# qdrant/quantization

Measured on AMD Instinct MI355X. Metric: scored vectors/sec, 10Mx768 u8 dot, higher is better.
Workload: dtype u8; 1 GPU; 10000000 x 768 store: f32 U[0,1) -> scalar u8 (dot); per step: encode_query + score_all over the shard; quantizer=u8, rows_per_gpu=10000000, dim=768, distance=dot, exchange=scores, gather_group=1, launch=single rank, world_size_seen=1, encode_ahead=False, total_rows=10000000, queries=16

## Files before the change

include/quantization_amd.h:

```cpp
#ifndef QUANTIZATION_AMD_H
#define QUANTIZATION_AMD_H

#include <stddef.h>
#include <stdint.h>

#ifdef __cplusplus
extern "C" {
#endif

#define QAMD_API __attribute__((visibility("default")))

typedef enum {
    QAMD_OK = 0,
    QAMD_ERR_IO = 1,
    QAMD_ERR_ENCODING = 2,
    QAMD_ERR_ARGUMENTS = 3,
    QAMD_ERR_STOPPED = 4,
    QAMD_ERR_OUT_OF_RANGE = 5,
    QAMD_ERR_DEVICE = 6
} qamd_status;

typedef enum { QAMD_DOT = 0, QAMD_L1 = 1, QAMD_L2 = 2 } qamd_distance;

typedef enum { QAMD_MEM_HOST = 0, QAMD_MEM_DEVICE = 1 } qamd_mem;

typedef struct {
    uint64_t dim;
    uint64_t count;
    int32_t distance_type;
    int32_t invert;
} qamd_vector_parameters;

typedef int (*qamd_stop_fn)(void *user);

QAMD_API const char *qamd_last_error(void);
QAMD_API const char *qamd_version(void);
QAMD_API int qamd_device_count(void);
QAMD_API qamd_status qamd_set_device(int device);
QAMD_API int qamd_get_device(void);
QAMD_API void qamd_thread_release(void);

typedef struct qamd_u8 qamd_u8;
typedef struct qamd_u8_query qamd_u8_query;

typedef struct {
    uint64_t actual_dim;
    float alpha;
    float offset;
    float multiplier;
    qamd_vector_parameters vector_parameters;
} qamd_u8_metadata;

QAMD_API uint64_t qamd_u8_quantized_vector_size(const qamd_vector_parameters *vp);
QAMD_API uint64_t qamd_u8_actual_dim(const qamd_vector_parameters *vp);

QAMD_API qamd_status qamd_u8_encode(const float *data, qamd_mem data_mem,
                                    const qamd_vector_parameters *vp, const float *quantile,
                                    const float *alpha_offset, qamd_stop_fn stop, void *stop_user,
                                    void *stream, qamd_u8 **out);

typedef struct qamd_u8_encoder qamd_u8_encoder;
QAMD_API qamd_status qamd_u8_encoder_begin(const qamd_vector_parameters *vp, const float *quantile,
                                           const float *alpha_offset, qamd_stop_fn stop, void *stop_user,
                                           void *stream, qamd_u8_encoder **out);
QAMD_API qamd_status qamd_u8_encoder_observe(qamd_u8_encoder *e, const float *batch, uint64_t n_rows,
                                             qamd_mem batch_mem);
QAMD_API qamd_status qamd_u8_encoder_push(qamd_u8_encoder *e, const float *batch, uint64_t n_rows,
                                          qamd_mem batch_mem);
QAMD_API qamd_status qamd_u8_encoder_finish(qamd_u8_encoder *e, qamd_u8 **out);
QAMD_API void qamd_u8_encoder_abort(qamd_u8_encoder *e);

QAMD_API qamd_status qamd_u8_find_min_max(const float *data, qamd_mem data_mem, uint64_t n_rows, uint64_t dim,
                                          void *stream, float *min, float *max);
QAMD_API qamd_status qamd_u8_find_quantile_interval(const float *data, qamd_mem data_mem, uint64_t count, uint64_t dim,
                                                    float quantile, void *stream, int *found, float *min, float *max);

QAMD_API qamd_status qamd_u8_from_rows(const uint8_t *rows, qamd_mem rows_mem,
                                       const qamd_u8_metadata *meta, void *stream, qamd_u8 **out);

QAMD_API qamd_status qamd_u8_export_rows(const qamd_u8 *h, uint8_t *rows, qamd_mem rows_mem,
                                         void *stream);
QAMD_API qamd_status qamd_u8_export_rows_range(const qamd_u8 *h, uint64_t first_row, uint64_t n_rows,
                                               uint8_t *rows, qamd_mem rows_mem, void *stream);
QAMD_API qamd_status qamd_u8_get_metadata(const qamd_u8 *h, qamd_u8_metadata *out);

QAMD_API qamd_status qamd_u8_save(const qamd_u8 *h, const char *data_path, const char *meta_path);
QAMD_API qamd_status qamd_u8_load(const char *data_path, const char *meta_path,
// ... 329 lines not shown
```

quantization_amd/csrc/common.hpp:

```cpp
#pragma once

#include <hip/hip_runtime.h>

#include <atomic>
#include <mutex>
#include <cstdarg>
#include <cstdint>
#include <cstdlib>
#include <cstdio>
#include <cstring>
#include <string>
#include <vector>

#include "json.hpp"

#include "../../include/quantization_amd.h"

namespace qamd {

std::string &last_error();
qamd_status fail(qamd_status st, const char *fmt, ...) __attribute__((format(printf, 2, 3)));

#define QAMD_HIP(expr)                                                                      \
    do {                                                                                    \
// ... 20 lines not shown
    DeviceGuard &operator=(const DeviceGuard &) = delete;
    qamd_status status() const { return st_; }

  private:
    int prev_ = -1;
    bool switched_ = false;
    qamd_status st_ = QAMD_OK;
};
#define QAMD_ON_DEVICE(dev)                  \
    ::qamd::DeviceGuard _qamd_dev_guard(dev); \
    QAMD_TRY(_qamd_dev_guard.status())

inline const char *dev_env(const char *name) {
#ifdef QAMD_DEV
    return getenv(name);
#else
    (void)name;
    return nullptr;
#endif
}
inline uint64_t dev_env_u64(const char *name, uint64_t dflt) {
    const char *e = dev_env(name);
    if (!e || !*e) return dflt;
    char *end = nullptr;
    const unsigned long long v = strtoull(e, &end, 10);
    return (*end == 0 && v > 0) ? (uint64_t)v : dflt;
}
inline uint64_t stage_bytes(uint64_t dflt) {
    static const uint64_t v = dev_env_u64("QAMD_DEV_STAGE_BYTES", 0);
    return v ? v : dflt;
}
inline bool host_whole_allowed() {
    static const bool on = [] { const char *e = dev_env("QAMD_DEV_HOST_WHOLE"); return !(e && e[0] == '0'); }();
    return on;
}
inline uint64_t pq_planar_max_rows() {
    static const uint64_t v = dev_env_u64("QAMD_DEV_PQ_PLANAR_ROWS", 1ull << 28);
    return v;
}
inline uint64_t pq_skew_max_rows() {
    static const uint64_t v = dev_env_u64("QAMD_DEV_PQ_SKEW_ROWS", 1ull << 30);
    return v;
}

class DeviceOnce {
  public:
    template <class F> qamd_status run(F &&setup) {
        int dev = 0;
        if (hipGetDevice(&dev) != hipSuccess || dev < 0 || dev > 63) return setup();
        const uint64_t bit = 1ull << dev;
        if (done_.load(std::memory_order_acquire) & bit) return QAMD_OK;
        std::lock_guard<std::mutex> g(mu_);
        if (done_.load(std::memory_order_relaxed) & bit) return QAMD_OK;
        const qamd_status st = setup();
        if (st == QAMD_OK) done_.fetch_or(bit, std::memory_order_release);
        return st;
    }

  private:
    std::atomic<uint64_t> done_{0};
    std::mutex mu_;
};
#define QAMD_LDS_OPT_IN(kernel, bytes)                                                                            \
    do {                                                                                                          \
        static ::qamd::DeviceOnce _qamd_once;                                                                     \
        QAMD_TRY(_qamd_once.run([]() -> qamd_status {                                                             \
// ... 105 lines not shown
```

quantization_amd/csrc/u8.hip:

```cpp
#include <algorithm>
#include <cmath>
#include <cstdlib>
#include <memory>
#include <vector>

#include "common.hpp"
#include "lists.hpp"
#include "multi_reduce.hpp"
#include "topk.hpp"
#include "topk_device.hpp"
#include "u8_internal.hpp"

#pragma clang fp contract(off)

using namespace qamd;

namespace {

constexpr int kBlock = 256;
constexpr int kScanBlock = 512;
constexpr uint64_t kRowPad = 1024;
constexpr uint64_t kQuantileSample = 100000;

enum Epilogue : int { EPI_POINT = 0, EPI_INTERNAL = 1 };
// ... 59 lines not shown
}
template <int G> __device__ __forceinline__ float avx2_lane_sum(uint32_t (&acc)[8]) {
    float f[8];
#pragma unroll
    for (int k = 0; k < 8; k++) f[k] = (float)(int32_t)group_sum<G>(acc[k]);
    float a0 = f[0] + f[4], a1 = f[1] + f[5], a2 = f[2] + f[6], a3 = f[3] + f[7];
    return (a0 + a2) + (a1 + a3);
}

__device__ __forceinline__ uint32_t f32_to_u8(float v, float alpha, float offset) {
    float x = (v - offset) / alpha;
    x = (x < 0.0f) ? 0.0f : x;
    x = (x > 127.0f) ? 127.0f : x;
    return (x != x) ? 0u : (uint32_t)x;
}

__device__ __forceinline__ bool quant_decided(float y) {
    constexpr float kBand = 3.0517578125e-05f;
    const float fr = __builtin_amdgcn_fractf(y);
    return (__builtin_fabsf(fr - 0.5f) <= 0.5f - kBand) || (__builtin_fabsf(y - 64.0f) >= 64.0f + kBand);
}
__device__ __forceinline__ uint32_t quant_code(float y) {
    return (uint32_t)__builtin_amdgcn_fmed3f(y, 0.0f, 127.0f);
}
__device__ __forceinline__ uint32_t f32x4_to_u8x4_fast(const float4 &f, float alpha, float offset, float r_alpha) {
    const float y0 = (f.x - offset) * r_alpha, y1 = (f.y - offset) * r_alpha, y2 = (f.z - offset) * r_alpha,
                y3 = (f.w - offset) * r_alpha;
    if (quant_decided(y0) && quant_decided(y1) && quant_decided(y2) && quant_decided(y3))
        return quant_code(y0) | (quant_code(y1) << 8) | (quant_code(y2) << 16) | (quant_code(y3) << 24);
    return f32_to_u8(f.x, alpha, offset) | (f32_to_u8(f.y, alpha, offset) << 8) | (f32_to_u8(f.z, alpha, offset) << 16) |
           (f32_to_u8(f.w, alpha, offset) << 24);
}

template <int G, int ITERS, int UNROLL, bool IS_L1, bool EXACT, bool FILTER>
__global__ __launch_bounds__(kScanBlock) void u8_scan_kernel(
    const uint4 *__restrict__ codes, const float *__restrict__ offsets,
    const uint4 *__restrict__ qcodes, const float *__restrict__ q_off_p, float multiplier,
    uint32_t n_rows, uint32_t row_chunks, float *__restrict__ out, TopkFilter filt) {
    constexpr int RW = 64 / G;
    constexpr int TILE = RW * UNROLL;
    const int lane = threadIdx.x & 63;
    const int sub = lane % G;
    const int rslot = lane / G;
    const uint64_t wave = ((uint64_t)blockIdx.x * kScanBlock + threadIdx.x) >> 6;
    const uint64_t base = wave * TILE;
    if (base >= n_rows) return;

    uint4 v[UNROLL][ITERS];
#pragma unroll
    for (int u = 0; u < UNROLL; u++) {
        const uint64_t row = base + u * RW + rslot;
        const uint4 *p = codes + row * row_chunks;
#pragma unroll
        for (int it = 0; it < ITERS; it++) {
            const uint32_t c = sub + it * G;
            if (EXACT) {
                v[u][it] = ld_nt(p + c);
            } else {
                const uint32_t cc = c < row_chunks ? c : row_chunks - 1;
                uint4 t = ld_nt(p + cc);
                const bool in = c < row_chunks;
                v[u][it] = make_uint4(in ? t.x : 0, in ? t.y : 0, in ? t.z : 0, in ? t.w : 0);
            }
        }
    }
    uint4 q[ITERS];
#pragma unroll
    for (int it = 0; it < ITERS; it++) {
        const uint32_t c = sub + it * G;
        if (EXACT) {
            q[it] = qcodes[c];
        } else {
            const uint4 t = qcodes[c < row_chunks ? c : row_chunks - 1];
            const bool in = c < row_chunks;
            q[it] = make_uint4(in ? t.x : 0, in ? t.y : 0, in ? t.z : 0, in ? t.w : 0);
        }
    }
    const float q_off = *q_off_p;
    constexpr int NGROUPS = (UNROLL + G - 1) / G;
    float v_off[NGROUPS];
#pragma unroll
    for (int g = 0; g < NGROUPS; g++)
        v_off[g] = offsets[base + (uint64_t)(g * G + sub) * RW + rslot];
    float mine = 0.0f;
    uint32_t pivot = 0;
    if (FILTER) pivot = *filt.pivot_key;
#pragma unroll
    for (int u = 0; u < UNROLL; u++) {
        uint32_t acc = 0;
#pragma unroll
        for (int it = 0; it < ITERS; it++)
            acc = IS_L1 ? sad16(v[u][it], q[it], acc) : dot16(v[u][it], q[it], acc);
        acc = group_sum<G>(acc);
        if (sub == (u % G)) mine = epilogue(multiplier, acc, q_off, v_off[u / G], 0.0f, EPI_POINT);
        if ((u % G) == G - 1 || u == UNROLL - 1) {
            constexpr int dummy = 0;
            (void)dummy;
            const int first = (u / G) * G;
            const uint64_t row = base + (uint64_t)(first + sub) * RW + rslot;
            if (sub <= u - first && row < n_rows) {
                if (FILTER) topk_offer(filt, pivot, mine, (uint32_t)row);
                else __builtin_nontemporal_store(mine, out + row);
            }
        }
    }
}

template <int G, int ITERS, int UNROLL, int NQ, bool IS_L1, bool EXACT, bool FILTER>
__global__ __launch_bounds__(kScanBlock) void u8_scan_multi_kernel(
    const uint4 *__restrict__ codes, const float *__restrict__ offsets, const uint8_t *__restrict__ qcodes,
    uint32_t q_pitch, const float *__restrict__ q_offs, uint32_t nq_valid ,
    float multiplier, uint32_t n_rows, uint32_t row_chunks, float *__restrict__ out ,
    uint64_t out_pitch, TopkFilterSlices slices) {
    static_assert(G >= NQ, "one lane of the row group per query");
    constexpr int RW = 64 / G;
    constexpr int TILE = RW * UNROLL;
    constexpr int TPW = NQ;
    const int lane = threadIdx.x & 63;
    const int sub = lane % G, rslot = lane / G;
    const uint64_t wave = ((uint64_t)blockIdx.x * kScanBlock + threadIdx.x) >> 6;
    if (wave * TILE * TPW >= n_rows) return;
    uint4 q[NQ][ITERS];
#pragma unroll
    for (int j = 0; j < NQ; j++) {
        const uint4 *qj = reinterpret_cast<const uint4 *>(qcodes + (size_t)((uint32_t)j < nq_valid ? j : nq_valid - 1) * q_pitch);
// ... 649 lines not shown
    }
}

__global__ __launch_bounds__(kBlock) void split_rows_kernel(const uint32_t *__restrict__ rows32,
                                                           uint64_t n_rows, uint32_t row_dwords,
                                                           uint32_t *__restrict__ codes32,
                                                           float *__restrict__ offsets) {
    const uint64_t total = n_rows * row_dwords;
    const uint64_t stride = (uint64_t)gridDim.x * kBlock;
    for (uint64_t t = (uint64_t)blockIdx.x * kBlock + threadIdx.x; t < total; t += stride) {
        uint64_t r = t / row_dwords;
        uint32_t k = (uint32_t)(t - r * row_dwords);
        uint32_t w = rows32[t];
        if (k == 0)
            offsets[r] = __uint_as_float(w);
        else
            codes32[r * (row_dwords - 1) + (k - 1)] = w;
    }
}

__global__ __launch_bounds__(kBlock) void join_rows_kernel(const uint32_t *__restrict__ codes32,
                                                          const float *__restrict__ offsets,
                                                          uint64_t n_rows, uint32_t row_dwords,
                                                          uint32_t *__restrict__ rows32) {
    const uint64_t total = n_rows * row_dwords;
    const uint64_t stride = (uint64_t)gridDim.x * kBlock;
    for (uint64_t t = (uint64_t)blockIdx.x * kBlock + threadIdx.x; t < total; t += stride) {
        uint64_t r = t / row_dwords;
        uint32_t k = (uint32_t)(t - r * row_dwords);
        rows32[t] = k == 0 ? __float_as_uint(offsets[r]) : codes32[r * (row_dwords - 1) + (k - 1)];
    }
}

int grid_for(uint64_t work_items, uint64_t per_block, int blocks_per_cu) {
    uint64_t want = (work_items + per_block - 1) / per_block;
    uint64_t cap = (uint64_t)device_info().cu_count * blocks_per_cu;
    if (want < 1) want = 1;
    return (int)(want > cap ? cap : want);
}

float host_multiplier(float alpha, int distance, int invert) {
    float m = distance == QAMD_DOT ? alpha * alpha : distance == QAMD_L1 ? alpha : -2.0f * alpha * alpha;
    return invert ? -m : m;
}

uint64_t actual_dim_of(uint64_t dim) { return dim + (16 - dim % 16) % 16; }

}


namespace {

qamd_status alloc_store(qamd_u8 *h) {
    h->padded_rows = round_up(h->count, kRowPad) + kRowPad;
    h->row_chunks = (uint32_t)(h->meta.actual_dim / 16);
    QAMD_TRY(h->codes.alloc_zero_tail(h->padded_rows * h->meta.actual_dim, h->count * h->meta.actual_dim));
    QAMD_TRY(h->offsets.alloc_zero_tail(h->padded_rows * sizeof(float), h->count * sizeof(float)));
    return QAMD_OK;
}

template <bool IS_L1> struct ScanLaunch {
    template <int G, int ITERS, int UNROLL>
    static void go(const qamd_u8 *h, const uint4 *qc, const float *qo, float *out, const TopkFilter *filt,
                   hipStream_t s) {
        constexpr int TILE = (64 / G) * UNROLL;
        const uint64_t waves = (h->count + TILE - 1) / TILE;
        const unsigned grid = (unsigned)((waves + kScanBlock / 64 - 1) / (kScanBlock / 64));
        const bool exact = h->row_chunks == (uint32_t)(G * ITERS);
#define QAMD_U8_GO(EX, FI)                                                                                  \
    hipLaunchKernelGGL((u8_scan_kernel<G, ITERS, UNROLL, IS_L1, EX, FI>), dim3(grid), dim3(kScanBlock), 0, s, \
                       h->codes.as<uint4>(), h->offsets.as<float>(), qc, qo, h->meta.multiplier,            \
                       (uint32_t)h->count, h->row_chunks, out, filt ? *filt : TopkFilter{})
        if (filt) {
            if (exact) QAMD_U8_GO(true, true);
            else QAMD_U8_GO(false, true);
        } else {
            if (exact) QAMD_U8_GO(true, false);
            else QAMD_U8_GO(false, false);
        }
#undef QAMD_U8_GO
    }
};

template <bool IS_L1>
bool launch_scan(const qamd_u8 *h, const uint4 *qc, const float *qo, float *out, const TopkFilter *filt,
                 hipStream_t s) {
    using L = ScanLaunch<IS_L1>;
    const uint32_t rc = h->row_chunks;
    if (rc == 1) return L::template go<1, 1, 4>(h, qc, qo, out, filt, s), true;
    if (rc == 2) return L::template go<2, 1, 4>(h, qc, qo, out, filt, s), true;
    if (rc <= 4) return L::template go<4, 1, 8>(h, qc, qo, out, filt, s), true;
    if (rc <= 8) return L::template go<8, 1, 8>(h, qc, qo, out, filt, s), true;
    switch ((rc + 15) / 16) {
        case 1: return L::template go<16, 1, 8>(h, qc, qo, out, filt, s), true;
        case 2: return L::template go<16, 2, 4>(h, qc, qo, out, filt, s), true;
        case 3: return L::template go<16, 3, 4>(h, qc, qo, out, filt, s), true;
        case 4: return L::template go<16, 4, 2>(h, qc, qo, out, filt, s), true;
        case 5: return L::template go<16, 5, 2>(h, qc, qo, out, filt, s), true;
        case 6: return L::template go<16, 6, 2>(h, qc, qo, out, filt, s), true;
        case 7: return L::template go<16, 7, 2>(h, qc, qo, out, filt, s), true;
        case 8: return L::template go<16, 8, 2>(h, qc, qo, out, filt, s), true;
        default: break;
    }
    return false;
}

template <bool IS_L1>
void launch_scan_generic(const qamd_u8 *h, const uint4 *qc, const float *qo, float *out, hipStream_t s) {
    uint64_t waves = (h->count + 3) / 4;
    unsigned grid = (unsigned)((waves + kBlock / 64 - 1) / (kBlock / 64));
    hipLaunchKernelGGL((u8_scan_generic_kernel<IS_L1>), dim3(grid), dim3(kBlock), 0, s,
                       h->codes.as<uint4>(), h->offsets.as<float>(), qc, qo, h->meta.multiplier,
                       (uint32_t)h->count, h->row_chunks, out);
}

template <bool IS_L1> struct SmallLaunch {
    template <int G, int ITERS>
    static qamd_status go(const qamd_u8 *h, const uint4 *qc, const float *qo, const FusedQuery *fq, const SmallTopkPlan &pl,
                          const SmallTopk &p, hipStream_t s) {
        const bool exact = h->row_chunks == (uint32_t)(G * ITERS);
        if constexpr (G * ITERS * 16 > (int)kFusedQueryDims + 15 * 16) {
            if (fq) return fail(QAMD_ERR_ARGUMENTS, "fused query does not fit the kernel arguments");
        } else if (fq) {
            QueryByValue qv;
            memcpy(qv.v, fq->values, (size_t)fq->qdim * 4);
            const qamd_vector_parameters &vp = h->meta.vector_parameters;
#define QAMD_U8_SMALL_FUSED(EX)                                                                                        \
    hipLaunchKernelGGL((u8_topk_small_fused_kernel<G, ITERS, IS_L1, EX>), dim3(pl.workgroups), dim3(1024), 0, s,          \
                       h->codes.as<uint4>(), h->offsets.as<float>(), qv, fq->qdim, (uint32_t)h->meta.actual_dim,         \
                       h->meta.alpha, h->meta.offset, vp.distance_type, vp.invert, fq->qbuf, h->meta.multiplier,           \
                       (uint32_t)h->count, h->row_chunks, pl.rows_per_wg, p)
            if (exact) QAMD_U8_SMALL_FUSED(true);
            else QAMD_U8_SMALL_FUSED(false);
#undef QAMD_U8_SMALL_FUSED
            QAMD_HIP(hipGetLastError());
            return QAMD_OK;
        }
#define QAMD_U8_SMALL(EX)                                                                                       \
    hipLaunchKernelGGL((u8_topk_small_kernel<G, ITERS, IS_L1, EX>), dim3(pl.workgroups), dim3(1024), 0, s,       \
                       h->codes.as<uint4>(), h->offsets.as<float>(), qc, qo, h->meta.multiplier, (uint32_t)h->count, \
                       h->row_chunks, pl.rows_per_wg, p)
        if (exact) QAMD_U8_SMALL(true);
        else QAMD_U8_SMALL(false);
#undef QAMD_U8_SMALL
        QAMD_HIP(hipGetLastError());
        return QAMD_OK;
    }
};

int small_group(uint32_t rc) { return rc == 1 ? 1 : rc == 2 ? 2 : rc <= 4 ? 4 : rc <= 8 ? 8 : rc <= 128 ? 16 : 0; }

template <bool IS_L1>
qamd_status launch_small(const qamd_u8 *h, const uint4 *qc, const float *qo, const FusedQuery *fq, const SmallTopkPlan &pl,
                         const SmallTopk &p, hipStream_t s) {
    using L = SmallLaunch<IS_L1>;
    const uint32_t rc = h->row_chunks;
    if (rc == 1) return L::template go<1, 1>(h, qc, qo, fq, pl, p, s);
    if (rc == 2) return L::template go<2, 1>(h, qc, qo, fq, pl, p, s);
    if (rc <= 4) return L::template go<4, 1>(h, qc, qo, fq, pl, p, s);
    if (rc <= 8) return L::template go<8, 1>(h, qc, qo, fq, pl, p, s);
    switch ((rc + 15) / 16) {
        case 1: return L::template go<16, 1>(h, qc, qo, fq, pl, p, s);
        case 2: return L::template go<16, 2>(h, qc, qo, fq, pl, p, s);
        case 3: return L::template go<16, 3>(h, qc, qo, fq, pl, p, s);
        case 4: return L::template go<16, 4>(h, qc, qo, fq, pl, p, s);
        case 5: return L::template go<16, 5>(h, qc, qo, fq, pl, p, s);
        case 6: return L::template go<16, 6>(h, qc, qo, fq, pl, p, s);
        case 7: return L::template go<16, 7>(h, qc, qo, fq, pl, p, s);
        case 8: return L::template go<16, 8>(h, qc, qo, fq, pl, p, s);
        default: break;
    }
    return fail(QAMD_ERR_ARGUMENTS, "no small top-k kernel for %u chunks", rc);
}

template <bool IS_L1, int G, int ITERS, int UNROLL, int NQ>
void launch_multi_shape(const qamd_u8 *h, const uint8_t *qcodes, uint64_t q_pitch, const float *q_offs, uint32_t nq_valid,
                        float *out, const TopkFilterSlices *slices, hipStream_t s) {
    constexpr int TILE = (64 / G) * UNROLL * NQ;
    const uint64_t waves = (h->count + TILE - 1) / TILE;
    const unsigned grid = (unsigned)((waves + kScanBlock / 64 - 1) / (kScanBlock / 64));
    const bool exact = h->row_chunks == (uint32_t)(G * ITERS);
#define QAMD_U8_MULTI(EX, FI)                                                                                      \
    hipLaunchKernelGGL((u8_scan_multi_kernel<G, ITERS, UNROLL, NQ, IS_L1, EX, FI>), dim3(grid), dim3(kScanBlock), 0, s, \
                       h->codes.as<uint4>(), h->offsets.as<float>(), qcodes, (uint32_t)q_pitch, q_offs, nq_valid,   \
                       h->meta.multiplier, (uint32_t)h->count, h->row_chunks, out, (uint64_t)h->count,             \
                       slices ? *slices : TopkFilterSlices{})
    if (slices) {
        if (exact) QAMD_U8_MULTI(true, true);
        else QAMD_U8_MULTI(false, true);
    } else {
        if (exact) QAMD_U8_MULTI(true, false);
        else QAMD_U8_MULTI(false, false);
    }
#undef QAMD_U8_MULTI
}

bool lane_order(const qamd_u8 *h) {
    return h->lane_mode == 1 && h->meta.vector_parameters.distance_type != QAMD_L1;
}

uint32_t multi_width(const qamd_u8 *h) {
    const uint32_t rc = h->row_chunks, iters = (rc + 15) / 16;
    const bool l1 = h->meta.vector_parameters.distance_type == QAMD_L1;
    if (rc < 9 || iters > 8 || lane_order(h)) return 0;
    return l1 && iters <= 3 ? 8 : iters <= 6 ? 4 : 2;
}

template <bool IS_L1>
bool launch_multi(const qamd_u8 *h, uint32_t nq_valid, const uint8_t *qcodes, uint64_t q_pitch, const float *q_offs,
                  float *out, const TopkFilterSlices *slices, hipStream_t s) {
    const uint32_t iters = (h->row_chunks + 15) / 16, width = multi_width(h);
    if (nq_valid < 2 || nq_valid > width) return false;
#define QAMD_U8_MULTI_IT(IT, UN)                                                                              \
    case IT:                                                                                                  \
        if constexpr (IS_L1 && IT <= 3) {                                                                     \
            if (nq_valid > 4) {                                                                               \
                launch_multi_shape<IS_L1, 16, IT, UN, 8>(h, qcodes, q_pitch, q_offs, nq_valid, out, slices, s); \
                return true;                                                                                  \
            }                                                                                                 \
        }                                                                                                     \
        if (nq_valid > 2) launch_multi_shape<IS_L1, 16, IT, UN, (IT <= 6 ? 4 : 2)>(h, qcodes, q_pitch, q_offs, nq_valid, out, slices, s); \
        else launch_multi_shape<IS_L1, 16, IT, UN, 2>(h, qcodes, q_pitch, q_offs, nq_valid, out, slices, s);  \
        return true;
    switch (iters) {
        QAMD_U8_MULTI_IT(1, 4) QAMD_U8_MULTI_IT(2, 2) QAMD_U8_MULTI_IT(3, 2) QAMD_U8_MULTI_IT(4, 2)
        QAMD_U8_MULTI_IT(5, 1) QAMD_U8_MULTI_IT(6, 1) QAMD_U8_MULTI_IT(7, 1) QAMD_U8_MULTI_IT(8, 1)
        default: break;
    }
#undef QAMD_U8_MULTI_IT
    return false;
}

bool fused_capable(const qamd_u8 *h) { return !lane_order(h) && h->row_chunks <= 128; }

bool u8_small_plan(const qamd_u8 *h, uint32_t k, SmallTopkPlan &plan) {
    const int g = small_group(h->row_chunks);
    if (!g || !fused_capable(h)) return false;
    const uint32_t tile = 2 * (64 / g);
    const uint32_t least = (uint32_t)std::max<uint64_t>(16 * tile, (128 * 1024) / std::max<uint64_t>(h->meta.actual_dim, 1));
    return small_topk_plan(h->count, k, tile, least, plan);
}

qamd_status scan_ptrs(const qamd_u8 *h, const uint4 *qc, const float *qo, float *out_dev, hipStream_t s,
                      const TopkFilter *filt = nullptr) {
    if (h->count == 0) return QAMD_OK;
    const bool is_l1 = h->meta.vector_parameters.distance_type == QAMD_L1;
    if (lane_order(h)) {
        uint64_t waves = (h->count + 3) / 4;
        unsigned grid = (unsigned)((waves + kBlock / 64 - 1) / (kBlock / 64));
        hipLaunchKernelGGL((u8_scan_avx2_lanes_kernel<true>), dim3(grid), dim3(kBlock), 0, s,
                           h->codes.as<uint4>(), h->offsets.as<float>(), qc, qo, h->meta.multiplier,
                           (uint32_t)h->count, h->row_chunks, out_dev);
    } else if (is_l1) {
        if (!launch_scan<true>(h, qc, qo, out_dev, filt, s)) launch_scan_generic<true>(h, qc, qo, out_dev, s);
    } else {
        if (!launch_scan<false>(h, qc, qo, out_dev, filt, s)) launch_scan_generic<false>(h, qc, qo, out_dev, s);
    }
    QAMD_HIP(hipGetLastError());
    return QAMD_OK;
}

qamd_status scan_into(const qamd_u8 *h, const qamd_u8_query *q, float *out_dev, hipStream_t s,
                      const TopkFilter *filt = nullptr) {
    return scan_ptrs(h, reinterpret_cast<const uint4 *>(q->buf.as<uint8_t>() + 16), q->buf.as<float>(), out_dev, s, filt);
}

qamd_status check_query(const qamd_u8 *h, const qamd_u8_query *q) {
    if (!h || !q) return fail(QAMD_ERR_ARGUMENTS, "null handle or query");
    if (q->actual_dim != h->meta.actual_dim)
        return fail(QAMD_ERR_ARGUMENTS, "query has %llu codes, store rows have %llu",
                    (unsigned long long)q->actual_dim, (unsigned long long)h->meta.actual_dim);
    return QAMD_OK;
}

template <bool IS_L1>
qamd_status launch_pairs(const qamd_u8 *h, const uint4 *qc, const float *qo, const uint8_t *q_batch, uint32_t q_pitch,
                         const float *q_offs, const uint32_t *lists, uint32_t n_lists, const uint32_t *list_rows, float diff,
                         int mode, const uint32_t *ids_dev, uint64_t n_ids, float *out_dev, hipStream_t s) {
    const uint64_t ppb = pairs_per_block(n_ids, 16);
// ... 332 lines not shown
            const uint64_t nr = std::min(batch_rows, count - r0);
            const float *src = nullptr;
            QAMD_TRY(batch_src(r0, nr, src));
            QAMD_TRY(acc.feed(src, nr * dim, s));
            if (data_mem == QAMD_MEM_HOST) QAMD_HIP(hipStreamSynchronize(s));
        }
        float mn, mx;
        QAMD_TRY(acc.result(s, mn, mx));
        alpha = (mx - mn) / 127.0f;
        offset = mn;
        if (quantile && !(count < 127 || *quantile >= 1.0f)) {
            bool found = false;
            float qmn = 0.0f, qmx = 0.0f;
            QAMD_TRY(quantile_interval_device(data, data_mem, count, dim, *quantile, s, found, qmn, qmx));
            if (found) {
                alpha = (qmx - qmn) / 127.0f;
                offset = qmn;
            }
        }
    }

    for (uint64_t r0 = 0; r0 < count; r0 += batch_rows) {
        if (stop && stop(stop_user)) return fail(QAMD_ERR_STOPPED, "Stopped");
        const uint64_t nr = std::min(batch_rows, count - r0);
        const float *src = nullptr;
        QAMD_TRY(batch_src(r0, nr, src));
        QAMD_TRY(launch_quantize(h.get(), src, nr, r0, alpha, offset, s));
        if (data_mem == QAMD_MEM_HOST || stop) QAMD_HIP(hipStreamSynchronize(s));
    }
    QAMD_HIP(hipStreamSynchronize(s));
    h->meta.alpha = alpha;
    h->meta.offset = offset;
    h->meta.multiplier = host_multiplier(alpha, vp->distance_type, vp->invert);
    *out = h.release();
    return QAMD_OK;
}

qamd_status qamd_u8_from_rows(const uint8_t *rows, qamd_mem rows_mem, const qamd_u8_metadata *meta,
                              void *stream, qamd_u8 **out) {
    if (!meta || !out) return fail(QAMD_ERR_ARGUMENTS, "null argument");
    const qamd_vector_parameters &vp = meta->vector_parameters;
    if (meta->actual_dim != actual_dim_of(vp.dim))
        return fail(QAMD_ERR_ARGUMENTS, "metadata actual_dim %llu does not match dim %llu",
                    (unsigned long long)meta->actual_dim, (unsigned long long)vp.dim);
    if (vp.count > 0xFFFFFFFFull) return fail(QAMD_ERR_ARGUMENTS, "count exceeds u32 row ids");
    if (vp.count > 0 && !rows) return fail(QAMD_ERR_ARGUMENTS, "rows is null");
    QAMD_ON_DEVICE(current_device());
    hipStream_t s = as_stream(stream);
    std::unique_ptr<qamd_u8> h(new qamd_u8);
    h->device = current_device();
    h->count = vp.count;
    h->meta = *meta;
    QAMD_TRY(alloc_store(h.get()));
    const uint64_t stride = meta->actual_dim + 4;
    const uint32_t row_dwords = (uint32_t)(stride / 4);
    const uint64_t batch_rows = std::max<uint64_t>(1, stage_bytes(256ull << 20) / stride);
    DevBuf stage;
    if (rows_mem == QAMD_MEM_HOST && vp.count)
        QAMD_TRY(stage.alloc(std::min<uint64_t>(batch_rows, vp.count) * stride));
    for (uint64_t r0 = 0; r0 < vp.count; r0 += batch_rows) {
        const uint64_t nr = std::min(batch_rows, vp.count - r0);
        const uint8_t *src = rows + r0 * stride;
        if (rows_mem == QAMD_MEM_HOST) {
            QAMD_TRY(copy_in(stage.ptr, src, QAMD_MEM_HOST, nr * stride, s));
            src = stage.as<uint8_t>();
        }
        int grid = grid_for(nr * row_dwords, kBlock * 4, 8);
        hipLaunchKernelGGL(split_rows_kernel, dim3(grid), dim3(kBlock), 0, s,
                           reinterpret_cast<const uint32_t *>(src), nr, row_dwords,
                           h->codes.as<uint32_t>() + r0 * (row_dwords - 1), h->offsets.as<float>() + r0);
        QAMD_HIP(hipGetLastError());
        if (rows_mem == QAMD_MEM_HOST) QAMD_HIP(hipStreamSynchronize(s));
    }
    QAMD_HIP(hipStreamSynchronize(s));
    *out = h.release();
    return QAMD_OK;
}

qamd_status qamd_u8_export_rows_range(const qamd_u8 *h, uint64_t first_row, uint64_t n_rows, uint8_t *rows,
                                      qamd_mem rows_mem, void *stream) {
    if (!h) return fail(QAMD_ERR_ARGUMENTS, "null handle");
    if (first_row > h->count || n_rows > h->count - first_row)
        return fail(QAMD_ERR_OUT_OF_RANGE, "rows [%llu, +%llu) out of range (count %llu)", (unsigned long long)first_row,
                    (unsigned long long)n_rows, (unsigned long long)h->count);
    if (n_rows == 0) return QAMD_OK;
    if (!rows) return fail(QAMD_ERR_ARGUMENTS, "rows is null");
    QAMD_ON_DEVICE(h->device);
    hipStream_t s = as_stream(stream);
    const uint64_t stride = h->meta.actual_dim + 4;
    const uint32_t row_dwords = (uint32_t)(stride / 4);
    const uint64_t batch_rows = std::max<uint64_t>(1, stage_bytes(256ull << 20) / stride);
    DevBuf stage;
    if (rows_mem == QAMD_MEM_HOST) QAMD_TRY(stage.alloc(std::min<uint64_t>(batch_rows, n_rows) * stride));
    for (uint64_t r0 = 0; r0 < n_rows; r0 += batch_rows) {
        const uint64_t nr = std::min(batch_rows, n_rows - r0), src_row = first_row + r0;
        uint8_t *dst = rows_mem == QAMD_MEM_HOST ? stage.as<uint8_t>() : rows + r0 * stride;
        int grid = grid_for(nr * row_dwords, kBlock * 4, 8);
        hipLaunchKernelGGL(join_rows_kernel, dim3(grid), dim3(kBlock), 0, s,
                           h->codes.as<uint32_t>() + src_row * (row_dwords - 1), h->offsets.as<float>() + src_row, nr,
                           row_dwords, reinterpret_cast<uint32_t *>(dst));
        QAMD_HIP(hipGetLastError());
        if (rows_mem == QAMD_MEM_HOST)
            QAMD_TRY(copy_out(rows + r0 * stride, QAMD_MEM_HOST, dst, nr * stride, s));
    }
    return QAMD_OK;
}

// ... 423 lines not shown
                    (unsigned long long)(e->pushed + n_rows), (unsigned long long)e->vp.count);
    QAMD_ON_DEVICE(e->device);
    QAMD_TRY(encoder_close_pass1(e));
    const uint64_t dim = e->vp.dim;
    const uint64_t piece_rows = std::max<uint64_t>(1, stage_bytes(kStagePieceBytes) / (dim * 4 + 1));
    for (uint64_t r = 0; r < n_rows; r += piece_rows) {
        const uint64_t nr = std::min(piece_rows, n_rows - r);
        const void *src = nullptr;
        bool staged = false;
        QAMD_TRY(local_view(batch + r * dim, batch_mem, nr * dim * 4, e->stage, e->stream, &src, &staged));
        QAMD_TRY(launch_quantize(e->h.get(), static_cast<const float *>(src), nr, e->pushed + r, e->alpha, e->offset,
                                 e->stream));
        if (staged) QAMD_HIP(hipStreamSynchronize(e->stream));
    }
    e->pushed += n_rows;
    return QAMD_OK;
}

qamd_status qamd_u8_encoder_finish(qamd_u8_encoder *e, qamd_u8 **out) {
    if (!e || !out) return fail(QAMD_ERR_ARGUMENTS, "null argument");
    std::unique_ptr<qamd_u8_encoder> own(e);
    if (e->pushed != e->vp.count)
        return fail(QAMD_ERR_ARGUMENTS, "Vector count %llu does not match vector parameters count %llu",
                    (unsigned long long)e->pushed, (unsigned long long)e->vp.count);
    QAMD_ON_DEVICE(e->device);
    QAMD_HIP(hipStreamSynchronize(e->stream));
    if (e->vp.count == 0) {
        e->h->meta.alpha = e->h->meta.offset = e->h->meta.multiplier = 0.0f;
    } else {
        e->h->meta.alpha = e->alpha;
        e->h->meta.offset = e->offset;
        e->h->meta.multiplier = host_multiplier(e->alpha, e->vp.distance_type, e->vp.invert);
    }
    *out = e->h.release();
    return QAMD_OK;
}

void qamd_u8_encoder_abort(qamd_u8_encoder *e) {
    if (!e) return;
    DeviceGuard g(e->device);
    (void)hipStreamSynchronize(e->stream);
    delete e;
}

}

namespace qamd {

qamd_status u8_minmax_range(const float *data, qamd_mem mem, uint64_t n_rows, uint64_t dim, hipStream_t s, float *mn,
                            float *mx) {
    MinMaxAcc acc;
    QAMD_TRY(acc.init(s));
    DevBuf stage;
    const uint64_t piece_rows = std::max<uint64_t>(1, stage_bytes(kStagePieceBytes) / std::max<uint64_t>(dim * 4, 1));
    for (uint64_t r = 0; r < n_rows && dim; r += piece_rows) {
        const uint64_t nr = std::min(piece_rows, n_rows - r);
        const void *src = nullptr;
        bool staged = false;
        QAMD_TRY(local_view(data + r * dim, mem, nr * dim * 4, stage, s, &src, &staged));
        QAMD_TRY(acc.feed(static_cast<const float *>(src), nr * dim, s));
        if (staged) QAMD_HIP(hipStreamSynchronize(s));
    }
    return acc.result(s, *mn, *mx);
}

qamd_status u8_quantile_interval(const float *data, qamd_mem mem, uint64_t count, uint64_t dim, float quantile,
// ... 126 lines not shown
                                          : launch_multi<false>(h, nq, qcodes, pitch, offsets_dev + q, o, nullptr, stream));
        if (ok) {
            q += nq;
        } else {
            QAMD_TRY(scan_ptrs(h, reinterpret_cast<const uint4 *>(qcodes), offsets_dev + q, o, stream));
            q += 1;
        }
    }
    QAMD_HIP(hipGetLastError());
    return QAMD_OK;
}

qamd_status u8_topk_single(const qamd_u8 *h, const uint8_t *codes_dev, const float *offset_dev, uint32_t k,
                           int largest, uint32_t *out_ids, float *out_scores, qamd_mem out_mem, hipStream_t stream) {
    return u8_topk_ptrs(h, codes_dev, offset_dev, k, largest, out_ids, out_scores, out_mem, stream, nullptr);
}

qamd_status u8_score_single(const qamd_u8 *h, const uint8_t *codes_dev, const float *offset_dev, float *out_dev,
                            hipStream_t stream) {
    return scan_ptrs(h, reinterpret_cast<const uint4 *>(codes_dev), offset_dev, out_dev, stream);
}

}

#ifdef QAMD_DEV
extern "C" __attribute__((visibility("default"))) void qamd_dev_u8_ptrs(const qamd_u8 *h, const void **codes,
                                                                        const void **offsets) {
    *codes = h->codes.ptr;
    *offsets = h->offsets.ptr;
}
extern "C" __attribute__((visibility("default"))) const void *qamd_dev_u8_query_ptr(const qamd_u8_query *q) {
    return q->buf.ptr;
}
#endif
```

quantization_amd/csrc/u8_internal.hpp:

```cpp
#pragma once
#include <atomic>
#include <mutex>

#include "common.hpp"
#include "lists.hpp"

struct qamd_u8 {
    int device = 0;
    qamd_u8_metadata meta{};
    uint64_t count = 0;
    uint64_t padded_rows = 0;
    uint32_t row_chunks = 0;
    int lane_mode = 0;
    qamd::DevBuf codes;
    qamd::DevBuf offsets;
    mutable std::mutex sample_mu;
    mutable qamd::DevBuf sample_codes, sample_offsets;
    mutable uint32_t sample_rows = 0;
};

struct qamd_u8_query {
    int device = 0;
    uint64_t actual_dim = 0;
    qamd::DevBuf buf;
    mutable qamd::ReadyEvent ready;
    mutable std::vector<float> host_f32;
    float alpha = 0.0f, offset = 0.0f;
    int distance = 0, invert = 0;
    mutable std::atomic<bool> deferred{false};
    mutable std::mutex encode_mu;
    bool pooled = false;
    mutable std::atomic<bool> async_used{false};
    ~qamd_u8_query() {
        if (pooled) qamd::query_buf_put(buf, !async_used.load(std::memory_order_relaxed) && ready.complete());
    }
};

namespace qamd {
qamd_status u8_minmax_range(const float *data, qamd_mem mem, uint64_t n_rows, uint64_t dim, hipStream_t s, float *mn,
                            float *mx);
qamd_status u8_quantile_interval(const float *data, qamd_mem mem, uint64_t count, uint64_t dim, float quantile,
                                 hipStream_t s, bool *found, float *mn, float *mx);
}

namespace qamd {
qamd_status u8_encode_queries_device(const qamd_u8 *h, const float *queries_dev, uint64_t n_queries, uint64_t qdim,
                                     uint8_t *codes_dev , uint64_t code_pitch,
                                     float *offsets_dev ,
// ... 25 lines not shown
```

Before: 9.085 billion vectors/s.

## Add 7-bit packed code image to shrink u8 scan bandwidth

At encode time, when every stored code fits in 7 bits, builds a second device image that moves the bits of the trailing chunks into the free high bit of the leading chunks. Rows then occupy 7/8 of the original chunk count. The single-query scan kernel gains a PACKED path for Dot and L2. It splits each word into its 7-bit part and its high bits and uses a shifted dot against extra query chunks, cutting bytes read per row in a memory-bound scan. The cost is extra device memory, a synchronous build step, and more ALU work per chunk; the multi-query and small-top-k kernels still read the unpacked codes.

```diff
diff --git a/include/quantization_amd.h b/include/quantization_amd.h
--- a/include/quantization_amd.h
+++ b/include/quantization_amd.h
@@ -53,6 +53,7 @@
 
 QAMD_API uint64_t qamd_u8_quantized_vector_size(const qamd_vector_parameters *vp);
 QAMD_API uint64_t qamd_u8_actual_dim(const qamd_vector_parameters *vp);
+
 
 QAMD_API qamd_status qamd_u8_encode(const float *data, qamd_mem data_mem,
                                     const qamd_vector_parameters *vp, const float *quantile,
diff --git a/quantization_amd/csrc/common.hpp b/quantization_amd/csrc/common.hpp
--- a/quantization_amd/csrc/common.hpp
+++ b/quantization_amd/csrc/common.hpp
@@ -76,6 +76,10 @@
 }
 inline bool host_whole_allowed() {
     static const bool on = [] { const char *e = dev_env("QAMD_DEV_HOST_WHOLE"); return !(e && e[0] == '0'); }();
+    return on;
+}
+inline bool u8_packed_allowed() {
+    static const bool on = [] { const char *e = dev_env("QAMD_DEV_U8_PACKED"); return !(e && e[0] == '0'); }();
     return on;
 }
 inline uint64_t pq_planar_max_rows() {
diff --git a/quantization_amd/csrc/u8.hip b/quantization_amd/csrc/u8.hip
--- a/quantization_amd/csrc/u8.hip
+++ b/quantization_amd/csrc/u8.hip
@@ -115,11 +115,12 @@
            (f32_to_u8(f.w, alpha, offset) << 24);
 }
 
-template <int G, int ITERS, int UNROLL, bool IS_L1, bool EXACT, bool FILTER>
+template <int G, int ITERS, int UNROLL, bool IS_L1, bool EXACT, bool FILTER, bool PACKED = false>
 __global__ __launch_bounds__(kScanBlock) void u8_scan_kernel(
     const uint4 *__restrict__ codes, const float *__restrict__ offsets,
     const uint4 *__restrict__ qcodes, const float *__restrict__ q_off_p, float multiplier,
-    uint32_t n_rows, uint32_t row_chunks, float *__restrict__ out, TopkFilter filt) {
+    uint32_t n_rows, uint32_t row_chunks, uint32_t n_extra, float *__restrict__ out, TopkFilter filt) {
+    static_assert(!(PACKED && IS_L1), "the packed image serves Dot and L2 only");
     constexpr int RW = 64 / G;
     constexpr int TILE = RW * UNROLL;
     const int lane = threadIdx.x & 63;
@@ -139,6 +140,8 @@
             const uint32_t c = sub + it * G;
             if (EXACT) {
                 v[u][it] = ld_nt(p + c);
+            } else if (PACKED) {
+                v[u][it] = ld_nt(p + (it < ITERS - 1 || c < row_chunks ? c : row_chunks - 1));
             } else {
                 const uint32_t cc = c < row_chunks ? c : row_chunks - 1;
                 uint4 t = ld_nt(p + cc);
@@ -159,6 +162,18 @@
             q[it] = make_uint4(in ? t.x : 0, in ? t.y : 0, in ? t.z : 0, in ? t.w : 0);
         }
     }
+    uint4 qx[PACKED ? ITERS : 1];
+    uint32_t qsh[PACKED ? ITERS : 1];
+    if (PACKED) {
+#pragma unroll
+        for (int it = 0; it < ITERS; it++) {
+            const uint32_t c = sub + it * G, e = c / 7;
+            const bool has = c < 7 * n_extra;
+            const uint4 t = qcodes[has ? row_chunks + e : 0];
+            qx[it] = make_uint4(has ? t.x : 0, has ? t.y : 0, has ? t.z : 0, has ? t.w : 0);
+            qsh[it] = 7 - (c - 7 * e);
+        }
+    }
     const float q_off = *q_off_p;
     constexpr int NGROUPS = (UNROLL + G - 1) / G;
     float v_off[NGROUPS];
@@ -172,8 +187,17 @@
     for (int u = 0; u < UNROLL; u++) {
         uint32_t acc = 0;
 #pragma unroll
-        for (int it = 0; it < ITERS; it++)
-            acc = IS_L1 ? sad16(v[u][it], q[it], acc) : dot16(v[u][it], q[it], acc);
+        for (int it = 0; it < ITERS; it++) {
+            if (PACKED) {
+                const uint4 &w = v[u][it];
+                const uint32_t hi = dot16(make_uint4(w.x & 0x80808080u, w.y & 0x80808080u, w.z & 0x80808080u,
+                                                     w.w & 0x80808080u), qx[it], 0);
+                acc = dot16(make_uint4(w.x & 0x7F7F7F7Fu, w.y & 0x7F7F7F7Fu, w.z & 0x7F7F7F7Fu, w.w & 0x7F7F7F7Fu),
+                            q[it], acc) + (hi >> qsh[it]);
+            } else {
+                acc = IS_L1 ? sad16(v[u][it], q[it], acc) : dot16(v[u][it], q[it], acc);
+            }
+        }
         acc = group_sum<G>(acc);
         if (sub == (u % G)) mine = epilogue(multiplier, acc, q_off, v_off[u / G], 0.0f, EPI_POINT);
         if ((u % G) == G - 1 || u == UNROLL - 1) {
@@ -889,6 +913,32 @@
     }
 }
 
+__global__ __launch_bounds__(kBlock) void u8_pack7_kernel(const uint4 *__restrict__ codes, uint64_t n_rows,
+                                                          uint32_t row_chunks, uint32_t pchunks, uint32_t n_extra,
+                                                          uint4 *__restrict__ packed, uint32_t *__restrict__ bad) {
+    const uint64_t total = n_rows * pchunks, stride = (uint64_t)gridDim.x * kBlock;
+    uint32_t high = 0;
+    for (uint64_t t = (uint64_t)blockIdx.x * kBlock + threadIdx.x; t < total; t += stride) {
+        const uint64_t r = t / pchunks;
+        const uint32_t j = (uint32_t)(t - r * pchunks);
+        const uint4 *row = codes + r * row_chunks;
+        const uint4 a = row[j];
+        uint32_t w[4] = {a.x & 0x7F7F7F7Fu, a.y & 0x7F7F7F7Fu, a.z & 0x7F7F7F7Fu, a.w & 0x7F7F7F7Fu};
+        high |= a.x | a.y | a.z | a.w;
+        if (j < 7 * n_extra) {
+            const uint4 x = row[pchunks + j / 7];
+            const uint32_t b = j % 7;
+            high |= x.x | x.y | x.z | x.w;
+            w[0] |= ((x.x >> b) & 0x01010101u) << 7;
+            w[1] |= ((x.y >> b) & 0x01010101u) << 7;
+            w[2] |= ((x.z >> b) & 0x01010101u) << 7;
+            w[3] |= ((x.w >> b) & 0x01010101u) << 7;
+        }
+        packed[t] = make_uint4(w[0], w[1], w[2], w[3]);
+    }
+    if (high & 0x80808080u) atomicOr(bad, 1u);
+}
+
 int grid_for(uint64_t work_items, uint64_t per_block, int blocks_per_cu) {
     uint64_t want = (work_items + per_block - 1) / per_block;
     uint64_t cap = (uint64_t)device_info().cu_count * blocks_per_cu;
@@ -916,24 +966,70 @@
     return QAMD_OK;
 }
 
+qamd_status build_packed(qamd_u8 *h, hipStream_t s) {
+    h->packed.release();
+    h->packed_chunks = 0;
+    const uint32_t rc = h->row_chunks, n_extra = rc / 8, pchunks = rc - n_extra;
+    if (!u8_packed_allowed() || h->count == 0 || rc < 8 || rc > 128 ||
+        h->meta.vector_parameters.distance_type == QAMD_L1)
+        return QAMD_OK;
+    const uint64_t bytes = h->padded_rows * pchunks * 16;
+    size_t free_b = 0, total_b = 0;
+    if (hipMemGetInfo(&free_b, &total_b) != hipSuccess || free_b < 2 * bytes) {
+        (void)hipGetLastError();
+        return QAMD_OK;
+    }
+    DevBuf img, bad;
+    const std::string err = last_error();
+    if (img.alloc_zero_tail(bytes, h->count * pchunks * 16) != QAMD_OK || bad.alloc(sizeof(uint32_t), true) != QAMD_OK) {
+        (void)hipGetLastError();
+        last_error() = err;
+        return QAMD_OK;
+    }
+    hipLaunchKernelGGL(u8_pack7_kernel, dim3(grid_for(h->count * pchunks, kBlock, 8)), dim3(kBlock), 0, s,
+                       h->codes.as<uint4>(), h->count, rc, pchunks, n_extra, img.as<uint4>(), bad.as<uint32_t>());
+    QAMD_HIP(hipGetLastError());
+    uint32_t high = 0;
+    QAMD_HIP(hipMemcpyAsync(&high, bad.ptr, sizeof(high), hipMemcpyDeviceToHost, s));
+    QAMD_HIP(hipStreamSynchronize(s));
+    if (high) return QAMD_OK;
+    h->packed = std::move(img);
+    h->packed_chunks = pchunks;
+    return QAMD_OK;
+}
+
 template <bool IS_L1> struct ScanLaunch {
     template <int G, int ITERS, int UNROLL>
-    static void go(const qamd_u8 *h, const uint4 *qc, const float *qo, float *out, const TopkFilter *filt,
-                   hipStream_t s) {
+    static void go(const qamd_u8 *h, bool packed, uint32_t chunks, const uint4 *qc, const float *qo, float *out,
+                   const TopkFilter *filt, hipStream_t s) {
         constexpr int TILE = (64 / G) * UNROLL;
         const uint64_t waves = (h->count + TILE - 1) / TILE;
         const unsigned grid = (unsigned)((waves + kScanBlock / 64 - 1) / (kScanBlock / 64));
-        const bool exact = h->row_chunks == (uint32_t)(G * ITERS);
-#define QAMD_U8_GO(EX, FI)                                                                                  \
-    hipLaunchKernelGGL((u8_scan_kernel<G, ITERS, UNROLL, IS_L1, EX, FI>), dim3(grid), dim3(kScanBlock), 0, s, \
-                       h->codes.as<uint4>(), h->offsets.as<float>(), qc, qo, h->meta.multiplier,            \
-                       (uint32_t)h->count, h->row_chunks, out, filt ? *filt : TopkFilter{})
+        const bool exact = chunks == (uint32_t)(G * ITERS);
+        const uint4 *codes = packed ? h->packed.as<uint4>() : h->codes.as<uint4>();
+        const uint32_t n_extra = h->row_chunks - chunks;
+#define QAMD_U8_GO(EX, FI, PK)                                                                                  \
+    hipLaunchKernelGGL((u8_scan_kernel<G, ITERS, UNROLL, IS_L1, EX, FI, PK>), dim3(grid),                      \
+                       dim3(kScanBlock), 0, s, codes, h->offsets.as<float>(), qc, qo, h->meta.multiplier,          \
+                       (uint32_t)h->count, chunks, n_extra, out, filt ? *filt : TopkFilter{})
+        if constexpr (!IS_L1) {
+            if (packed) {
+                if (filt) {
+                    if (exact) QAMD_U8_GO(true, true, true);
+                    else QAMD_U8_GO(false, true, true);
+                } else {
+                    if (exact) QAMD_U8_GO(true, false, true);
+                    else QAMD_U8_GO(false, false, true);
+                }
+                return;
+            }
+        }
         if (filt) {
-            if (exact) QAMD_U8_GO(true, true);
-            else QAMD_U8_GO(false, true);
+            if (exact) QAMD_U8_GO(true, true, false);
+            else QAMD_U8_GO(false, true, false);
         } else {
-            if (exact) QAMD_U8_GO(true, false);
-            else QAMD_U8_GO(false, false);
+            if (exact) QAMD_U8_GO(true, false, false);
+            else QAMD_U8_GO(false, false, false);
         }
 #undef QAMD_U8_GO
     }
@@ -943,20 +1039,22 @@
 bool launch_scan(const qamd_u8 *h, const uint4 *qc, const float *qo, float *out, const TopkFilter *filt,
                  hipStream_t s) {
     using L = ScanLaunch<IS_L1>;
-    const uint32_t rc = h->row_chunks;
-    if (rc == 1) return L::template go<1, 1, 4>(h, qc, qo, out, filt, s), true;
-    if (rc == 2) return L::template go<2, 1, 4>(h, qc, qo, out, filt, s), true;
-    if (rc <= 4) return L::template go<4, 1, 8>(h, qc, qo, out, filt, s), true;
-    if (rc <= 8) return L::template go<8, 1, 8>(h, qc, qo, out, filt, s), true;
+    const bool packed = !IS_L1 && h->packed_chunks != 0;
+    const uint32_t rc = packed ? h->packed_chunks : h->row_chunks;
+    h->last_scan_packed.store(packed ? 1 : 0, std::memory_order_relaxed);
+    if (rc == 1) return L::template go<1, 1, 4>(h, packed, rc, qc, qo, out, filt, s), true;
+    if (rc == 2) return L::template go<2, 1, 4>(h, packed, rc, qc, qo, out, filt, s), true;
+    if (rc <= 4) return L::template go<4, 1, 8>(h, packed, rc, qc, qo, out, filt, s), true;
+    if (rc <= 8) return L::template go<8, 1, 8>(h, packed, rc, qc, qo, out, filt, s), true;
     switch ((rc + 15) / 16) {
-        case 1: return L::template go<16, 1, 8>(h, qc, qo, out, filt, s), true;
-        case 2: return L::template go<16, 2, 4>(h, qc, qo, out, filt, s), true;
-        case 3: return L::template go<16, 3, 4>(h, qc, qo, out, filt, s), true;
-        case 4: return L::template go<16, 4, 2>(h, qc, qo, out, filt, s), true;
-        case 5: return L::template go<16, 5, 2>(h, qc, qo, out, filt, s), true;
-        case 6: return L::template go<16, 6, 2>(h, qc, qo, out, filt, s), true;
-        case 7: return L::template go<16, 7, 2>(h, qc, qo, out, filt, s), true;
-        case 8: return L::template go<16, 8, 2>(h, qc, qo, out, filt, s), true;
+        case 1: return L::template go<16, 1, 8>(h, packed, rc, qc, qo, out, filt, s), true;
+        case 2: return L::template go<16, 2, 4>(h, packed, rc, qc, qo, out, filt, s), true;
+        case 3: return L::template go<16, 3, 4>(h, packed, rc, qc, qo, out, filt, s), true;
+        case 4: return L::template go<16, 4, 2>(h, packed, rc, qc, qo, out, filt, s), true;
+        case 5: return L::template go<16, 5, 2>(h, packed, rc, qc, qo, out, filt, s), true;
+        case 6: return L::template go<16, 6, 2>(h, packed, rc, qc, qo, out, filt, s), true;
+        case 7: return L::template go<16, 7, 2>(h, packed, rc, qc, qo, out, filt, s), true;
+        case 8: return L::template go<16, 8, 2>(h, packed, rc, qc, qo, out, filt, s), true;
         default: break;
     }
     return false;
@@ -1012,6 +1110,7 @@
                          const SmallTopk &p, hipStream_t s) {
     using L = SmallLaunch<IS_L1>;
     const uint32_t rc = h->row_chunks;
+    h->last_scan_packed.store(0, std::memory_order_relaxed);
     if (rc == 1) return L::template go<1, 1>(h, qc, qo, fq, pl, p, s);
     if (rc == 2) return L::template go<2, 1>(h, qc, qo, fq, pl, p, s);
     if (rc <= 4) return L::template go<4, 1>(h, qc, qo, fq, pl, p, s);
@@ -1037,6 +1136,7 @@
     const uint64_t waves = (h->count + TILE - 1) / TILE;
     const unsigned grid = (unsigned)((waves + kScanBlock / 64 - 1) / (kScanBlock / 64));
     const bool exact = h->row_chunks == (uint32_t)(G * ITERS);
+    h->last_scan_packed.store(0, std::memory_order_relaxed);
 #define QAMD_U8_MULTI(EX, FI)                                                                                      \
     hipLaunchKernelGGL((u8_scan_multi_kernel<G, ITERS, UNROLL, NQ, IS_L1, EX, FI>), dim3(grid), dim3(kScanBlock), 0, s, \
                        h->codes.as<uint4>(), h->offsets.as<float>(), qcodes, (uint32_t)q_pitch, q_offs, nq_valid,   \
@@ -1102,6 +1202,7 @@
                       const TopkFilter *filt = nullptr) {
     if (h->count == 0) return QAMD_OK;
     const bool is_l1 = h->meta.vector_parameters.distance_type == QAMD_L1;
+    h->last_scan_packed.store(0, std::memory_order_relaxed);
     if (lane_order(h)) {
         uint64_t waves = (h->count + 3) / 4;
         unsigned grid = (unsigned)((waves + kBlock / 64 - 1) / (kBlock / 64));
@@ -1500,6 +1601,7 @@
     h->meta.alpha = alpha;
     h->meta.offset = offset;
     h->meta.multiplier = host_multiplier(alpha, vp->distance_type, vp->invert);
+    QAMD_TRY(build_packed(h.get(), s));
     *out = h.release();
     return QAMD_OK;
 }
@@ -1541,6 +1643,7 @@
         if (rows_mem == QAMD_MEM_HOST) QAMD_HIP(hipStreamSynchronize(s));
     }
     QAMD_HIP(hipStreamSynchronize(s));
+    QAMD_TRY(build_packed(h.get(), s));
     *out = h.release();
     return QAMD_OK;
 }
@@ -2030,6 +2133,7 @@
         e->h->meta.offset = e->offset;
         e->h->meta.multiplier = host_multiplier(e->alpha, e->vp.distance_type, e->vp.invert);
     }
+    QAMD_TRY(build_packed(e->h.get(), e->stream));
     *out = e->h.release();
     return QAMD_OK;
 }
@@ -2222,4 +2326,12 @@
 extern "C" __attribute__((visibility("default"))) const void *qamd_dev_u8_query_ptr(const qamd_u8_query *q) {
     return q->buf.ptr;
 }
+extern "C" __attribute__((visibility("default"))) void qamd_dev_u8_packed(const qamd_u8 *h, const void **packed,
+                                                                          uint32_t *chunks) {
+    *packed = h->packed.ptr;
+    *chunks = h->packed_chunks;
+}
+extern "C" __attribute__((visibility("default"))) int qamd_dev_u8_last_scan_packed(const qamd_u8 *h) {
+    return h->last_scan_packed.load(std::memory_order_relaxed);
+}
 #endif
diff --git a/quantization_amd/csrc/u8_internal.hpp b/quantization_amd/csrc/u8_internal.hpp
--- a/quantization_amd/csrc/u8_internal.hpp
+++ b/quantization_amd/csrc/u8_internal.hpp
@@ -14,6 +14,9 @@
     int lane_mode = 0;
     qamd::DevBuf codes;
     qamd::DevBuf offsets;
+    qamd::DevBuf packed;
+    uint32_t packed_chunks = 0;
+    mutable std::atomic<int> last_scan_packed{0};
     mutable std::mutex sample_mu;
     mutable qamd::DevBuf sample_codes, sample_offsets;
     mutable uint32_t sample_rows = 0;
```

After: 9.810 billion vectors/s, median of 6. 8.0% higher.
